# mhauskn/dqn-hfo

Measured on AMD Instinct MI355X. Metric: DQN updates/sec, 1v0 HFO, 4x1024 MLP, minibatch 256, higher is better.
Workload: dtype f32; 1 GPU; BASELINE configs[1]: 1v0 HFO, 1 MI355X, 4x1024 actor-critic, minibatch 256, 1M-transition device replay; replay_transitions=1000000, state_size=58, minibatch=256, minibatch_per_gpu=256, global_minibatch=256, parallelism=single, hip_graph=True, prewarm_updates=992, tuning_flags=0, sampling=on-device Philox, uniform with replacement

## Files before the change

__graft_entry__.py:

```python
import importlib.util
import os
import sys

ROOT = os.path.dirname(os.path.abspath(__file__))


def load_package():
    if "dqn_hfo_amd" in sys.modules:
        return sys.modules["dqn_hfo_amd"]
    pkg_dir = os.path.join(ROOT, "dqn-hfo_amd")
    spec = importlib.util.spec_from_file_location(
        "dqn_hfo_amd", os.path.join(pkg_dir, "__init__.py"), submodule_search_locations=[pkg_dir])
    mod = importlib.util.module_from_spec(spec)
    sys.modules["dqn_hfo_amd"] = mod
    spec.loader.exec_module(mod)
    return mod


def build():
    pkg = load_package()
    lib = pkg.build(verbose=False)
    assert os.path.exists(lib), lib
    if ROOT not in sys.path:
        sys.path.insert(0, ROOT)
    from oracle import c_oracle
    c_oracle.build()
    pkg.capi.load()
    sys.path.insert(0, os.path.join(ROOT, "tests"))
    import testlib
    testlib.load_test()
    from oracle import dropin_build
    if dropin_build.reference_present():
        dropin_build.build(lib)
    return lib


def smoke():
    import numpy as np
    pkg = load_package()
    if ROOT not in sys.path:
        sys.path.insert(0, ROOT)
    sys.path.insert(0, os.path.join(ROOT, "tests"))
    from oracle import c_oracle, torch_ref
    from synth import synth_replay
    rng = np.random.default_rng(7)
    B, S, hid = 32, 59, (128, 64, 64, 64)
    dqn = pkg.DQN(S, minibatch=B, hidden=hid, memory=4096, seed=3)
    orc = c_oracle.Oracle(B=B, S=S, hidden=hid, capacity=4096)
    for net, actor in ((0, True), (1, False)):
        w = torch_ref.init_params_np(rng, S, hid, actor) * 10
        dqn.set_params(net, w); dqn.CloneNet(net)
        orc.set_params(net, w); orc.clone_to_target(net)
    s, a, r, mc, nx, term = synth_replay(rng, 1024, S, mean_len=10)
    dqn.add_transitions_arrays(s, a, r, mc, nx, term)
    orc.add_transitions(s, a, r, mc, nx, term)
    for it in range(3):
        idx = rng.integers(0, 1024, size=B)
        l1, q1 = dqn.UpdateActorCritic(idx)
        l2, q2 = orc.update(idx)
        assert abs(l1 - l2) <= 1e-4 * max(1.0, abs(l2)), (l1, l2)
        assert abs(q1 - q2) <= 1e-4, (q1, q2)
    for net in range(4):
        d = np.abs(dqn.get_params(net) - orc.get_params(net)).max()
# ... 15 lines not shown
```

benchlib/flops.py:

```python


HBM_PEAK_GBS = 8000.0


MFMA_F32_PEAK_TF = 157.3


def tower_weights(in_dim, hidden):
    dims = (in_dim,) + tuple(hidden)
    return [dims[i] * dims[i + 1] for i in range(len(hidden))]


def family_flops(B, S, hidden, shifted=True):
    wa = tower_weights(S, hidden)
    wc = tower_weights(S + 10, hidden)
    h1 = hidden[0]
    L = len(hidden)
    if shifted and L >= 2:
        pair = lambda w: sum(w[j + 1] + w[j] for j in range(1, L - 1))
        return {
            "gemm_fwd_lds_4x2": 2 * B * (2 * sum(wa[1:]) + 2 * sum(wc[1:])),
            "gemm_fwd_lds_2x2": 2 * B * sum(wc[1:]),
            "gemm_fwd_direct": 2 * B * (2 * wa[0] + 3 * wc[0]),
            "gemm_bwd_pair": 2 * B * (pair(wc) + pair(wa)),
            "gemm_dgrad": 2 * B * (sum(wc[1:]) + 10 * h1 + wc[L - 1] + wa[L - 1]),
            "gemm_wgrad": 2 * B * (wc[1] + wc[0] + wa[1] + wa[0]),
        }
    return {
        "gemm_fwd_lds_4x2": 2 * B * (2 * sum(wa[1:]) + 2 * sum(wc[1:])),
        "gemm_fwd_lds_2x2": 2 * B * sum(wc[1:]),
        "gemm_fwd_direct": 2 * B * (2 * wa[0] + 3 * wc[0]),
        "gemm_bwd_pair": 2 * B * (2 * sum(wc[1:]) + 2 * sum(wa[1:])),
        "gemm_dgrad": 2 * B * (sum(wc[1:]) + 10 * h1),
        "gemm_wgrad": 2 * B * (wc[0] + wa[0]),
    }


def family_flops16(B, S, hidden):
    wa = tower_weights(S, hidden)
    wc = tower_weights(S + 10, hidden)
    h1 = hidden[0]
    return {
        "hgemm_fwd": 2 * B * (2 * sum(wa) + 3 * sum(wc)),
        "hgemm_dgrad": 2 * B * (sum(wc[1:]) + sum(wa[1:]) + sum(wc[1:]) + 10 * h1),
        "hgemm_wgrad": 2 * B * (sum(wc) + sum(wa)),
    }


MFMA_F16_PEAK_TF = 2500.0


KERNEL_NAMES = {"hgemm_fwd": "hgemm_nt<2,2>/<1,1> (forward epilogue)", "hgemm_dgrad": "hgemm_nt (dgrad epilogue)",
                "hgemm_wgrad": "hgemm_nt (wgrad epilogue)","gemm_fwd_lds_4x2": "gemm_fwd_lds<4,2,true,1>", "gemm_fwd_lds_2x2": "gemm_fwd_lds<2,2,true,2>",
                "gemm_fwd_direct": "gemm_fwd_direct<4,2>", "gemm_bwd_pair": "gemm_bwd_seq<true>",
                "gemm_dgrad": "gemm_dgrad_lds<1,1>", "gemm_wgrad": "gemm_wgrad_tail<1>"}


TRACE_FAMILY = (("gemm_fwd_lds<4,2,true,1>", "gemm_fwd_lds_4x2"), ("gemm_fwd_lds<4,2,true>", "gemm_fwd_lds_4x2"), ("gemm_fwd_lds<2,2,true", "gemm_fwd_lds_2x2"),
                ("gemm_fwd_lds<1,1,true", "gemm_fwd_lds_2x2"), ("gemm_fwd_direct", "gemm_fwd_direct"), ("gemm_bwd_seq", "gemm_bwd_pair"),
                ("gemm_bwd_pair_direct", "gemm_bwd_pair"), ("gemm_dgrad_lds", "gemm_dgrad"), ("gemm_dgrad_direct", "gemm_dgrad"), ("gemm_dgrad_narrow", "gemm_dgrad"), ("k_dqda_head_bwd", "gemm_dgrad"), ("k_dgrad_qtrain", "gemm_dgrad"),
                ("gemm_wgrad_tail", "gemm_wgrad"), ("gemm_wgrad_narrow", "gemm_wgrad"), ("k_adam_soft", "adam"))
```

dqn-hfo_amd/capi.py:

```python
import ctypes as C
import os

from ._build import LIB, build

MAX_HIDDEN = 8
DP_ID_BYTES = 128
DP_PER_LAYER, DP_HALF_GRADS, DP_SHARD_OPT = 1, 2, 4
DP_UNVERIFIED_OK = 256
TUNE_FP16_WGRAD_PER_LAYER = 1
TUNE_SEPARATE_HEAD_SEED = 2
TUNE_BWD_UNSHIFTED = 4
TUNE_SEPARATE_ACTOR_HEAD_BWD = 8
TUNE_SEPARATE_Q_TRAIN = 16
TUNE_SEPARATE_FIRST_LAYER = 32
TUNE_SEPARATE_CRITIC_FIRST_LAYERS = 64
TUNE_LATE_GATHER = 128
PLAN_FORMS = ("fp16", "data_parallel", "bwd_shifted_critic", "bwd_shifted_actor", "head_wgrad_rides_critic", "head_wgrad_rides_actor",
              "q_train_in_dgrad", "head_seed_fused", "dqda_head_bwd", "critic_l0_rides", "first_layers_merged", "early_gather_l0", "dp_tails_ride", "prioritized")
LOSS_SCALE_STATIC, LOSS_SCALE_DYNAMIC = 0, 1
FP32, FP16 = 0, 1
ACTOR, CRITIC, ACTOR_TARGET, CRITIC_TARGET = 0, 1, 2, 3
KIND_W, KIND_M, KIND_V, KIND_G = 0, 1, 2, 3


class Config(C.Structure):
    _fields_ = [
        ("struct_size", C.c_int32), ("minibatch", C.c_int32), ("state_size", C.c_int32),
        ("num_hidden", C.c_int32), ("hidden", C.c_int32 * MAX_HIDDEN),
        ("replay_capacity", C.c_int32), ("soft_update_freq", C.c_int32),
        ("gamma", C.c_double), ("beta", C.c_double), ("tau", C.c_double),
        ("actor_lr", C.c_float), ("critic_lr", C.c_float), ("momentum", C.c_float),
        ("momentum2", C.c_float), ("delta", C.c_float), ("clip_gradients", C.c_float),
        ("device", C.c_int32), ("dp_world", C.c_int32), ("dp_rank", C.c_int32), ("use_graph", C.c_int32),
        ("seed", C.c_uint64), ("stream", C.c_void_p), ("grad_arena", C.c_void_p),
        ("grad_arena_bytes", C.c_size_t), ("precision", C.c_int32), ("loss_scale", C.c_float),
        ("tuning_flags", C.c_int32),
        ("loss_scale_mode", C.c_int32), ("loss_scale_growth_interval", C.c_int32),
        ("loss_scale_min_mult", C.c_float), ("loss_scale_max_mult", C.c_float),
    ]


class LossScaleState(C.Structure):
    _fields_ = [("struct_size", C.c_int32), ("mode", C.c_int32), ("mult_critic", C.c_float), ("mult_actor", C.c_float),
                ("good_critic", C.c_int32), ("good_actor", C.c_int32), ("backoffs_critic", C.c_int32), ("backoffs_actor", C.c_int32),
                ("growths_critic", C.c_int32), ("growths_actor", C.c_int32), ("skipped_steps", C.c_int32), ("reserved", C.c_int32)]


class UpdatePlan(C.Structure):
    _fields_ = [("struct_size", C.c_int32), ("forms", C.c_int32), ("launches_single", C.c_int32), ("launches_graph_first", C.c_int32),
# ... 169 lines not shown
```

dqn-hfo_amd/csrc/gemm_bodies.hip.h:

```cpp
#pragma once
#include <hip/hip_runtime.h>

#include <cstdint>

#include "learner_args.hip.h"

namespace dqnhip {


__host__ __device__ __forceinline__ void tile_of_counts(int tiles_p, int tiles_q, int b, int& tile_p, int& tile_q) {
  const bool xmap = (tiles_p & 7) == 0;
  const int j = xmap ? b >> 3 : b;
  const int d = j / tiles_q;
  tile_q = j - d * tiles_q;
  tile_p = xmap ? d * 8 + (b & 7) : d;
}
__device__ __forceinline__ void tile_of_problem(const GemmProblem& pr, int b, int& tile_p, int& tile_q) {
  tile_of_counts(pr.tiles_p, pr.tiles_q, b, tile_p, tile_q);
}
__device__ __forceinline__ void tile_of_block(const GemmBatch& batch, int& pi, int& tile_p, int& tile_q) {
  int b = blockIdx.x;
  pi = 0;
#pragma unroll
  for (int i = 1; i < kMaxGroup; ++i)
// ... 370 lines not shown
#define DN_COMPUTE(slot)                                                                \
  { _Pragma("unroll") for (int s = 0; s < 4; ++s) acc[0] = DQN_MFMA((float)rp[slot][s], (float)rq[slot][s], acc[0]); }
  const int nkbN = nkb - nkb % NS;
  if (nkbN > 0) {
#pragma unroll
    for (int i = 0; i < NS; ++i) { DN_LOAD(i, i) DQN_PIN(); }
    int kb = 0;
    for (; kb + NS < nkbN; kb += NS) {
#pragma unroll
      for (int i = 0; i < NS; ++i) { DN_COMPUTE(i) DQN_PIN(); DN_LOAD(i, kb + NS + i) DQN_PIN(); }
    }
#pragma unroll
    for (int i = 0; i < NS; ++i) { DN_COMPUTE(i) }
  }
  for (int kb = nkbN; kb < nkb; ++kb) { DN_LOAD(0, kb) DN_COMPUTE(0) }
#undef DN_LOAD
#undef DN_COMPUTE
  park_accumulators<1>(smem, acc, wave, lane);
  __syncthreads();
  f32x4 v = f32x4{0.f, 0.f, 0.f, 0.f};
  if (wave == 0) v = reduce_accumulator<1>(smem, 0, lane);
  return v;
}
__device__ __forceinline__ void dgrad_narrow_body(const GemmProblem& pr, int tile_p, int tile_q, float* smem) {
  const f32x4 v = dgrad_narrow_tile<4>(pr, tile_p, tile_q, smem);
  if ((threadIdx.x >> 6) == 0) {
    const int lane = threadIdx.x & 63, li = lane & 15, lg = lane >> 4;
    const int q = tile_q * 16 + li, p = tile_p * 16 + (lg << 2);
    *reinterpret_cast<f32x4*>(pr.C + (size_t)q * pr.ldc + p) = v;
  }
}

constexpr int kWgradRing = 4;
template <int TPB, int TQB>
__device__ __forceinline__ void wgrad_direct_body(const GemmProblem& pr, int tile_p, int tile_q, float* smem) {
  constexpr int NACC = TPB * 4 * TQB * 4;
  const int lane = threadIdx.x & 63, wave = threadIdx.x >> 6;
  const int li = lane & 15, lg = lane >> 4;
  const int p0 = tile_p * 64 * TPB, q0 = tile_q * 64 * TQB;
  const int Kw = pr.Kred >> 2;
  const int nst = Kw >> 2;
  const float* pp = pr.P + (size_t)(wave * Kw + lg) * pr.ldp + p0 + li * 4;
  const float* qp = pr.Q + (size_t)(wave * Kw + lg) * pr.ldq + q0 + li * 4;
  const size_t ldp = pr.ldp, ldq = pr.ldq;
  const bool want_db = (pr.db != nullptr) && (tile_p == 0);

  f32x4 acc[NACC];
#pragma unroll
  for (int e = 0; e < NACC; ++e) acc[e] = f32x4{0.f, 0.f, 0.f, 0.f};
  f32x4 dbacc[TQB];
#pragma unroll
  for (int d = 0; d < TQB; ++d) dbacc[d] = f32x4{0.f, 0.f, 0.f, 0.f};
  constexpr int NS = kWgradRing;
  f32x4 rp[NS][TPB], rq[NS][TQB];

#define WG_LOAD(slot, st)                                                               \
  {                                                                                     \
    _Pragma("unroll") for (int b = 0; b < TPB; ++b)                                     \
        rp[slot][b] = *reinterpret_cast<const f32x4*>(pp + (size_t)((st) << 2) * ldp + b * 64); \
    _Pragma("unroll") for (int d = 0; d < TQB; ++d)                                     \
        rq[slot][d] = *reinterpret_cast<const f32x4*>(qp + (size_t)((st) << 2) * ldq + d * 64); \
  }
#define WG_COMPUTE(slot)                                                                \
  {                                                                                     \
    _Pragma("unroll") for (int d = 0; d < TQB; ++d) {                                   \
      dbacc[d].x += rq[slot][d].x; dbacc[d].y += rq[slot][d].y;                         \
      dbacc[d].z += rq[slot][d].z; dbacc[d].w += rq[slot][d].w;                         \
      _Pragma("unroll") for (int qc = 0; qc < 4; ++qc)                                  \
// ... 10 lines not shown
    for (int i = 0; i < NS; ++i) { WG_LOAD(i, i) DQN_PIN(); }
    int st = 0;
    for (; st + NS < nstN; st += NS) {
#pragma unroll
      for (int i = 0; i < NS; ++i) { WG_COMPUTE(i) DQN_PIN(); WG_LOAD(i, st + NS + i) DQN_PIN(); }
    }
#pragma unroll
    for (int i = 0; i < NS; ++i) { WG_COMPUTE(i) }
  }
  {
    const int rem = nst - nstN;
    if (rem > 0) WG_LOAD(0, nstN)
    if (rem > 1) WG_LOAD(1, nstN + 1)
    if (rem > 2) WG_LOAD(2, nstN + 2)
    if (rem > 0) WG_COMPUTE(0)
    if (rem > 1) WG_COMPUTE(1)
    if (rem > 2) WG_COMPUTE(2)
  }
#undef WG_LOAD
#undef WG_COMPUTE

  park_accumulators<NACC>(smem, acc, wave, lane);
  float* sdb = smem + 4 * NACC * 64 * 4;
  if (want_db) {
#pragma unroll
    for (int d = 0; d < TQB; ++d) {
      f32x4 v = dbacc[d];
      v.x += __shfl_xor(v.x, 16, 64); v.y += __shfl_xor(v.y, 16, 64); v.z += __shfl_xor(v.z, 16, 64); v.w += __shfl_xor(v.w, 16, 64);
      v.x += __shfl_xor(v.x, 32, 64); v.y += __shfl_xor(v.y, 32, 64); v.z += __shfl_xor(v.z, 32, 64); v.w += __shfl_xor(v.w, 32, 64);
      if (lg == 0) reinterpret_cast<f32x4*>(sdb)[(wave * TQB + d) * 16 + li] = v;
    }
  }
  __syncthreads();
  float ssq = 0.0f;
#pragma unroll
  for (int g4 = 0; g4 < TQB * 4 * TPB; ++g4) {
    if ((g4 & 3) == wave) {
      const int b = g4 % TPB, dq = g4 / TPB, qc = dq & 3, d = dq >> 2;
      f32x4 r0 = reduce_accumulator<NACC>(smem, g4 * 4 + 0, lane);
      f32x4 r1 = reduce_accumulator<NACC>(smem, g4 * 4 + 1, lane);
      f32x4 r2 = reduce_accumulator<NACC>(smem, g4 * 4 + 2, lane);
      f32x4 r3 = reduce_accumulator<NACC>(smem, g4 * 4 + 3, lane);
      const int n = q0 + d * 64 + (li << 2) + qc;
#pragma unroll
      for (int r = 0; r < 4; ++r) {
        const int p = p0 + b * 64 + (lg << 4) + (r << 2);
        const f32x4 v = f32x4{r0[r], r1[r], r2[r], r3[r]};
        ssq = fmaf(v.x, v.x, ssq); ssq = fmaf(v.y, v.y, ssq); ssq = fmaf(v.z, v.z, ssq); ssq = fmaf(v.w, v.w, ssq);
        *reinterpret_cast<f32x4*>(pr.C + (size_t)n * pr.ldc + p) = v;
      }
    }
  }
  if (want_db && wave == 0 && lane < 16 * TQB) {
    const int d = lane >> 4, l16 = lane & 15;
    const f32x4* s4 = reinterpret_cast<const f32x4*>(sdb);
    const f32x4 a0 = s4[(0 * TQB + d) * 16 + l16], a1 = s4[(1 * TQB + d) * 16 + l16];
    const f32x4 a2 = s4[(2 * TQB + d) * 16 + l16], a3 = s4[(3 * TQB + d) * 16 + l16];
    f32x4 v;
    v.x = (a0.x + a1.x) + (a2.x + a3.x); v.y = (a0.y + a1.y) + (a2.y + a3.y);
    v.z = (a0.z + a1.z) + (a2.z + a3.z); v.w = (a0.w + a1.w) + (a2.w + a3.w);
    *reinterpret_cast<f32x4*>(pr.db + q0 + d * 64 + (l16 << 2)) = v;
    ssq = fmaf(v.x, v.x, ssq); ssq = fmaf(v.y, v.y, ssq); ssq = fmaf(v.z, v.z, ssq); ssq = fmaf(v.w, v.w, ssq);
  }
  if (pr.partial != nullptr) {
    ssq = wave_sum64(ssq);
    __syncthreads();
// ... 461 lines not shown
```

dqn-hfo_amd/csrc/gemm_direct.hip.h:

```cpp
#pragma once
#include <hip/hip_runtime.h>

#include <algorithm>
#include <cstdint>
#include <cstdlib>

#include "gemm_bodies.hip.h"
#include "gemm_plan.hip.h"

namespace dqnhip {

template <int TP, int TQ>
__global__ __launch_bounds__(256) void gemm_fwd_direct(const GemmArgs<kMaxGroup> args) {
  extern __shared__ __attribute__((aligned(16))) float smem[];
  int tile_p, tile_q;
  const GemmProblem pr = problem_of_block(args, tile_p, tile_q);
  fwd_direct_body<TP, TQ>(pr, tile_p, tile_q, smem);
}
template <int TP, int TQ, bool PIN, int NSLOT = 2>
__global__ __launch_bounds__(256) void gemm_fwd_lds(const GemmArgs<kMaxGroup> args) {
  extern __shared__ __attribute__((aligned(16))) float smem[];
  int tile_p, tile_q;
  const GemmProblem pr = problem_of_block(args, tile_p, tile_q);
  fwd_lds_body<TP, TQ, PIN, NSLOT>(pr, tile_p, tile_q, smem);
// ... 50 lines not shown
}
template <int TQD = 1, bool DLDS = false>
__global__ __launch_bounds__(256) void gemm_bwd_pair_direct(const GemmArgs<kMaxGroup> args) {
  extern __shared__ __attribute__((aligned(16))) float smem[];
  int tile_p, tile_q;
  const GemmProblem pr = problem_of_block(args, tile_p, tile_q);
  if (pr.mode == GEMM_WGRAD) wgrad_direct_body<1, 1>(pr, tile_p, tile_q, smem);
  else if constexpr (DLDS) dgrad_lds_body<1, TQD, false>(pr, tile_p, tile_q, smem);
  else dgrad_direct_body<1, TQD>(pr, tile_p, tile_q, smem);
}

template <bool DLDS>
__device__ __forceinline__ void bwd_seq_block(const GemmArgs<2>& args, const int block, float* smem) {
  int tile_p, tile_q;
  HotArgs<2> r;
  const int b = request_args(args, r, block);
  const GemmProblem pw = problem_at<1>(args, r);
  if (b < pw.tiles_p * pw.tiles_q) {
    tile_of_problem(pw, b, tile_p, tile_q);
    wgrad_direct_body<1, 1>(pw, tile_p, tile_q, smem);
  }
  __syncthreads();
  const GemmProblem pd = problem_at<0>(args, r);
  if (b < pd.tiles_p * pd.tiles_q) {
    tile_of_problem(pd, b, tile_p, tile_q);
    if constexpr (DLDS) dgrad_lds_body<1, 1, true>(pd, tile_p, tile_q, smem);
    else dgrad_direct_body<1, 1>(pd, tile_p, tile_q, smem);
  }
}
template <bool DLDS>
__global__ __launch_bounds__(256) void gemm_bwd_seq(const GemmArgs<2> args) {
  extern __shared__ __attribute__((aligned(16))) float smem[];
  bwd_seq_block<DLDS>(args, (int)blockIdx.x, smem);
}

template <int NH>
__global__ __launch_bounds__(256) void gemm_wgrad_narrow_rider(const GemmArgs<kMaxGroup> args, const HeadWgradRider rider) {
  extern __shared__ __attribute__((aligned(16))) float smem[];
  HotArgs<kMaxGroup> r;
  const int b = request_args(args, r, (int)blockIdx.x, rider.blocks);
  if (b < rider.blocks) { head_wgrad_rider<NH>(rider, b, smem); return; }
  int tile_p, tile_q;
  const GemmProblem pr = problem_of_tile(args, r, b - rider.blocks, tile_p, tile_q);
  wgrad_narrow_body<1>(pr, tile_p, tile_q, smem);
}

template <int NH>
__global__ __launch_bounds__(256) void gemm_wgrad_tail(const GemmArgs<2> args, const HeadWgradRider rider, const TailsArgs tails) {
  extern __shared__ __attribute__((aligned(16))) float smem[];
  HotArgs<2> r;
  int blk = request_args(args, r, (int)blockIdx.x, tails.on, rider.blocks);
  int tile_p, tile_q;
  if (tails.on && blk == tails.on - 1) { tails_block(tails, smem, reinterpret_cast<double*>(smem + 8)); return; }
  if (blk < rider.blocks) { head_wgrad_rider<NH>(rider, blk, smem); return; }
  blk -= rider.blocks;
  const int n0 = r.hd.tiles_p[1] * r.hd.tiles_q[1];
  if (blk < n0) { const GemmProblem p0 = problem_at<1>(args, r); tile_of_problem(p0, blk, tile_p, tile_q); wgrad_narrow_body<1>(p0, tile_p, tile_q, smem); return; }
  blk -= n0;
  const GemmProblem p1 = problem_at<0>(args, r);
  tile_of_problem(p1, blk, tile_p, tile_q); wgrad_direct_body<1, 1>(p1, tile_p, tile_q, smem);
}


constexpr int kBwdTileLds = 4 * 16 * 64 * 16 + 4 * 16 * 16;
constexpr int kWgradTailLdsMax = 80 * 1024;

// ... 109 lines not shown
template <int NH>
inline hipError_t wgrad_narrow_rider_launch(GemmBatch& batch, const HeadWgradRider& rider, const LaunchOn& on) {
  const size_t lds = std::max(head_rider_lds_bytes<NH>(rider), (size_t)wgrad_narrow_lds_bytes<1>());
  if (lds > 64 * 1024) return hipErrorInvalidValue;
  tile_batch(batch, 64, 16);
  return packed_launch(gemm_wgrad_narrow_rider<NH>, batch, rider.blocks, (int)lds, on, rider);
}
template <int NH>
inline hipError_t wgrad_tail_launch(GemmBatch& batch, const HeadWgradRider& rider, const LaunchOn& on, const TailsArgs* tails_in = nullptr) {
  TailsArgs tails{}; if (tails_in != nullptr) { tails = *tails_in; tails.on = 1; }
  GemmProblem& w1 = batch.prob[0]; GemmProblem& w0 = batch.prob[1];
  w1.tiles_p = w1.Pdim / 64; w1.tiles_q = w1.Qdim / 64; w1.tile_base = 0;
  w0.tiles_p = w0.Pdim / 64; w0.tiles_q = w0.Qdim / 16; w0.tile_base = w1.tiles_p * w1.tiles_q;
  const int grid = w0.tile_base + w0.tiles_p * w0.tiles_q + rider.blocks + (tails.on ? 1 : 0);
  batch.total_tiles = grid;
  if (tails.on) tails.on = grid;
  const size_t lds = std::max(rider.blocks ? head_rider_lds_bytes<NH>(rider) : (size_t)0, (size_t)kBwdTileLds);
  if (lds > (size_t)kWgradTailLdsMax) return hipErrorInvalidValue;
  GemmArgs<2> args;
  if (batch.n != 2 || !pack_args(batch, args)) return hipErrorInvalidValue;
  return launch(on, gemm_wgrad_tail<NH>, dim3(grid), dim3(256), lds, args, rider, tails);
}
template <bool DLDS>
inline hipError_t bwd_seq_launch(GemmBatch& batch, const LaunchOn& on) {
  GemmProblem& d = batch.prob[0]; GemmProblem& w = batch.prob[1];
  d.tiles_p = d.Pdim / 64; d.tiles_q = d.Qdim / 16; d.tile_base = 0;
  w.tiles_p = w.Pdim / 64; w.tiles_q = w.Qdim / 64; w.tile_base = 0;
  const int nd = d.tiles_p * d.tiles_q, nw = w.tiles_p * w.tiles_q;
  const int grid = nd > nw ? nd : nw;
  batch.total_tiles = grid;
  GemmArgs<2> args;
  if (batch.n != 2 || !pack_args(batch, args, false)) return hipErrorInvalidValue;
  return launch(on, gemm_bwd_seq<DLDS>, dim3(grid), dim3(256), kBwdTileLds, args);
}
template <int UNUSED = 0>
inline hipError_t gemm_form_launch(int form, GemmBatch& b, const LaunchOn& on, const HeadWgradRider* rider = nullptr, const TailsArgs* tails = nullptr) {
  if (!gemm_form_accepts(form, b)) return hipErrorInvalidValue;
  const bool tail = form == GEMM_FORM_WGRAD_TAIL_1 || form == GEMM_FORM_WGRAD_TAIL_NO;
  if (!tail && (rider != nullptr || tails != nullptr)) return hipErrorInvalidValue;
  const HeadWgradRider no_rider{};
  switch (form) {
    case GEMM_FORM_FWD_DIRECT_2x2: return fwd_direct_launch<2, 2>(b, on);
    case GEMM_FORM_FWD_DIRECT_4x2: return fwd_direct_launch<4, 2>(b, on);
    case GEMM_FORM_FWD_LDS_1x1: return fwd_lds_launch<1, 1, true>(b, on);
    case GEMM_FORM_FWD_LDS_2x2: return fwd_lds_launch<2, 2, true>(b, on);
    case GEMM_FORM_FWD_LDS_4x2: return fwd_lds_launch<4, 2, true>(b, on);
    case GEMM_FORM_FWD_LDS_4x2_ONE_IMAGE: return fwd_lds_launch<4, 2, true, 1>(b, on);
    case GEMM_FORM_DGRAD_DIRECT: return dgrad_direct_launch<1, 1>(b, on);
    case GEMM_FORM_DGRAD_LDS: return dgrad_lds_launch<1, 1>(b, on);
    case GEMM_FORM_DGRAD_NARROW: return dgrad_narrow_launch(b, on);
    case GEMM_FORM_WGRAD_NARROW: return wgrad_narrow_launch<1>(b, on);
    case GEMM_FORM_BWD_SEQ: return bwd_seq_launch<false>(b, on);
    case GEMM_FORM_BWD_SEQ_LDS: return bwd_seq_launch<true>(b, on);
    case GEMM_FORM_BWD_PAIR: return bwd_pair_direct_launch<1, false>(b, on);
    case GEMM_FORM_BWD_PAIR_LDS: return bwd_pair_direct_launch<1, true>(b, on);
    case GEMM_FORM_WGRAD_TAIL_1: return wgrad_tail_launch<1>(b, rider ? *rider : no_rider, on, tails);
    case GEMM_FORM_WGRAD_TAIL_NO: return wgrad_tail_launch<kNO>(b, rider ? *rider : no_rider, on, tails);
  }
  return hipErrorInvalidValue;
}
template <typename K>
inline hipError_t direct_prepare(K kernel, int lds_bytes) {
  return hipFuncSetAttribute(reinterpret_cast<const void*>(kernel), hipFuncAttributeMaxDynamicSharedMemorySize, lds_bytes);
}
template <int UNUSED = 0>
inline hipError_t direct_prepare_all() {
  hipError_t e = direct_prepare(gemm_bwd_seq<true>, kBwdTileLds);
  if (e == hipSuccess) e = direct_prepare(gemm_bwd_seq<false>, kBwdTileLds);
  if (e == hipSuccess) e = direct_prepare(gemm_wgrad_tail<1>, kWgradTailLdsMax);
  if (e == hipSuccess) e = direct_prepare(gemm_wgrad_tail<10>, kWgradTailLdsMax);
  if (e == hipSuccess) e = direct_prepare(gemm_bwd_pair_direct<1, true>, kBwdTileLds);
  if (e == hipSuccess) e = direct_prepare(gemm_bwd_pair_direct<1, false>, kBwdTileLds);
  if (e == hipSuccess) e = direct_prepare(gemm_fwd_lds<4, 2, true>, fwd_lds_bytes<4, 2, true>());
  return e;
}

}
```

dqn-hfo_amd/csrc/gemm_plan.hip.h:

```cpp
#pragma once
#include "gemm_common.hip.h"

namespace dqnhip {

enum GemmForm {
  GEMM_FORM_FWD_DIRECT_2x2 = 0, GEMM_FORM_FWD_DIRECT_4x2 = 1,
  GEMM_FORM_FWD_LDS_1x1 = 2, GEMM_FORM_FWD_LDS_2x2 = 3, GEMM_FORM_FWD_LDS_4x2 = 4, GEMM_FORM_FWD_LDS_4x2_ONE_IMAGE = 5,
  GEMM_FORM_DGRAD_DIRECT = 6, GEMM_FORM_DGRAD_LDS = 7, GEMM_FORM_DGRAD_NARROW = 8, GEMM_FORM_WGRAD_NARROW = 9,
  GEMM_FORM_BWD_SEQ = 10, GEMM_FORM_BWD_SEQ_LDS = 11,
  GEMM_FORM_BWD_PAIR = 12, GEMM_FORM_BWD_PAIR_LDS = 13,
  GEMM_FORM_WGRAD_TAIL_1 = 14, GEMM_FORM_WGRAD_TAIL_NO = 15,
  GEMM_FORM_COUNT = 16
};
enum GemmFormKind { GEMM_KIND_FWD_DIRECT, GEMM_KIND_FWD_LDS, GEMM_KIND_DGRAD, GEMM_KIND_DGRAD_NARROW, GEMM_KIND_WGRAD_NARROW,
                    GEMM_KIND_BWD , GEMM_KIND_TAIL };
struct GemmFormSpec { GemmFormKind kind; int bp, bq; bool lds; int n_min, n_max; const char* name; };
inline constexpr GemmFormSpec kGemmForms[GEMM_FORM_COUNT] = {
    {GEMM_KIND_FWD_DIRECT, 32, 32, false, 1, kMaxGroup, "fwd_direct<2,2>"},
    {GEMM_KIND_FWD_DIRECT, 64, 32, false, 1, kMaxGroup, "fwd_direct<4,2>"},
    {GEMM_KIND_FWD_LDS, 16, 16, true, 1, kMaxGroup, "fwd_lds<1,1,true>"},
    {GEMM_KIND_FWD_LDS, 32, 32, true, 1, kMaxGroup, "fwd_lds<2,2,true>"},
    {GEMM_KIND_FWD_LDS, 64, 32, true, 1, kMaxGroup, "fwd_lds<4,2,true>"},
    {GEMM_KIND_FWD_LDS, 64, 32, true, 1, kMaxGroup, "fwd_lds<4,2,true,1>"},
    {GEMM_KIND_DGRAD, 64, 16, false, 1, kMaxGroup, "dgrad_direct<1,1>"},
// ... 19 lines not shown
inline bool gemm_fwd_accepts(const GemmProblem& p, const GemmFormSpec& f) {
  if (p.mode != GEMM_FWD || !gemm_tiles_ok(p, f.bp, f.bq) || !gemm_kred_ok(p.Kred, f.lds)) return false;
  if (p.mask || p.db || p.partial) return false;
  if (p.xcopy_dst && (f.lds || p.xcopy_n <= 0 || p.xcopy_col < 0 || (long)p.xcopy_col + p.xcopy_n > p.ldp)) return false;
  return !p.seed_w == !p.C2 && !p.dot_w == !p.dot_out;
}
inline bool gemm_dgrad_accepts(const GemmProblem& p, bool lds, bool narrow) {
  if (p.mode != GEMM_DGRAD || !gemm_tiles_ok(p, narrow ? 16 : 64, 16) || !gemm_kred_ok(p.Kred, lds)) return false;
  return gemm_fwd_extras_absent(p) && !p.db && !p.partial;
}
inline bool gemm_wgrad_accepts(const GemmProblem& p, bool narrow) {
  if (p.mode != GEMM_WGRAD || !gemm_tiles_ok(p, 64, narrow ? 16 : 64) || p.Kred < 16 || p.Kred % 16) return false;
  return gemm_fwd_extras_absent(p) && !p.mask;
}
inline bool gemm_form_accepts(int form, const GemmBatch& b) {
  if (form < 0 || form >= GEMM_FORM_COUNT) return false;
  const GemmFormSpec& f = kGemmForms[form];
  if (b.n < f.n_min || b.n > f.n_max) return false;
  switch (f.kind) {
    case GEMM_KIND_FWD_DIRECT: case GEMM_KIND_FWD_LDS:
      for (int i = 0; i < b.n; ++i) if (!gemm_fwd_accepts(b.prob[i], f)) return false;
      return true;
    case GEMM_KIND_DGRAD: case GEMM_KIND_DGRAD_NARROW:
      for (int i = 0; i < b.n; ++i) if (!gemm_dgrad_accepts(b.prob[i], f.lds, f.kind == GEMM_KIND_DGRAD_NARROW)) return false;
      return true;
    case GEMM_KIND_WGRAD_NARROW:
      for (int i = 0; i < b.n; ++i) if (!gemm_wgrad_accepts(b.prob[i], true)) return false;
      return true;
    case GEMM_KIND_BWD: return gemm_dgrad_accepts(b.prob[0], f.lds, false) && gemm_wgrad_accepts(b.prob[1], false);
    case GEMM_KIND_TAIL: return gemm_wgrad_accepts(b.prob[0], false) && gemm_wgrad_accepts(b.prob[1], true);
  }
  return false;
}

inline GemmForm fwd_form(int kred, int pdim, int rows, int n) {
  const bool lds = gemm_lds_ok(kred);
  if (n == 1) {
    if (lds && rows <= 128) return GEMM_FORM_FWD_LDS_1x1;
    if (lds && rows >= 512 && pdim % 64 == 0) return GEMM_FORM_FWD_LDS_4x2;
    return lds ? GEMM_FORM_FWD_LDS_2x2 : GEMM_FORM_FWD_DIRECT_2x2;
  }
  const long t42 = (long)n * (pdim / 64) * (rows / 32), t22 = (long)n * (pdim / 32) * (rows / 32);
  if (lds) {
    if (t42 >= 192) return GEMM_FORM_FWD_LDS_4x2_ONE_IMAGE;
    if (t22 >= 128 || rows > 128 || rows % 16) return GEMM_FORM_FWD_LDS_2x2;
    return GEMM_FORM_FWD_LDS_1x1;
  }
  return t42 >= 64 ? GEMM_FORM_FWD_DIRECT_4x2 : GEMM_FORM_FWD_DIRECT_2x2;
}
inline GemmForm first_layers_form() { return GEMM_FORM_FWD_DIRECT_4x2; }

inline bool bwd_layer_is_pair(int kp_in, int out, int rows) {
  const long tiles = (long)(kp_in / 64) * (rows / 16) + (long)(kp_in / 64) * (out / 64);
  return tiles <= 256 && rows % 16 == 0 && kp_in % 64 == 0 && out % 64 == 0;
}
inline GemmForm dgrad_form(int out, bool narrow = false) {
  return narrow ? GEMM_FORM_DGRAD_NARROW : (gemm_lds_ok(out) ? GEMM_FORM_DGRAD_LDS : GEMM_FORM_DGRAD_DIRECT);
}
inline GemmForm wgrad_form() { return GEMM_FORM_WGRAD_NARROW; }
inline GemmForm bwd_form(int kp_in, int out, int rows) {
  if (bwd_layer_is_pair(kp_in, out, rows)) return gemm_lds_ok(out) ? GEMM_FORM_BWD_PAIR_LDS : GEMM_FORM_BWD_PAIR;
  return gemm_lds_ok(out) ? GEMM_FORM_BWD_SEQ_LDS : GEMM_FORM_BWD_SEQ;
}
inline GemmForm bwd_shifted_mid_form(int out) { return gemm_lds_ok(out) ? GEMM_FORM_BWD_SEQ_LDS : GEMM_FORM_BWD_SEQ; }
inline GemmForm bwd_shifted_tail_form(int nh) { return nh == 1 ? GEMM_FORM_WGRAD_TAIL_1 : GEMM_FORM_WGRAD_TAIL_NO; }

}
```

dqn-hfo_amd/csrc/learner.hip:

```cpp
#include "learner_internal.hip.h"
#include "gemm_direct.hip.h"
#include "hgemm.hip.h"
#include "head_fwd_kernels.hip.h"
#include "head_kernels.hip.h"
#include "small_kernels.hip.h"

using namespace dqnhip;
using namespace dqnhip_host;

namespace dqnhip_host {

const char* const kFamily[kNumFamily] = {"gemm_fwd_lds_4x2", "gemm_dgrad", "gemm_wgrad", "adam", "gemm_bwd_pair", "gemm_fwd_lds_2x2", "gemm_fwd_direct",
                                         "hgemm_fwd", "hgemm_dgrad", "hgemm_wgrad",
                                         "per_sync", "per_sample", "per_update"};
static Family family_of(GemmForm f, int n) {
  switch (kGemmForms[f].kind) {
    case GEMM_KIND_FWD_DIRECT: return kFamFwdDirect;
    case GEMM_KIND_FWD_LDS: return n == 1 ? kFamFwdLds2x2 : kFamFwdLds4x2;
    case GEMM_KIND_DGRAD: case GEMM_KIND_DGRAD_NARROW: return kFamDgrad;
    case GEMM_KIND_BWD: return kFamBwdPair;
    case GEMM_KIND_WGRAD_NARROW: case GEMM_KIND_TAIL: break;
  }
  return kFamWgrad;
}
// ... 43 lines not shown
    p.P = wat(h, net, l.w_off[i]); p.ldp = l.kp[i];
    p.Q = dZ[i + 1]; p.ldq = l.kp[i + 1];
    p.C = dZ[i]; p.ldc = l.kp[i];
    p.Pdim = l.kp[i]; p.Qdim = rows; p.Kred = l.dims[i + 1];
    p.mask = i > 0 ? act[i] : nullptr; p.ldm = l.kp[i];
    return p;
  };
  auto wgrad_of = [&](int i) {
    GemmProblem p{};
    p.mode = GEMM_WGRAD;
    p.P = act[i]; p.ldp = l.kp[i];
    p.Q = dZ[i + 1]; p.ldq = l.kp[i + 1];
    p.C = garena + l.w_off[i]; p.ldc = l.kp[i];
    p.Pdim = l.kp[i]; p.Qdim = l.dims[i + 1]; p.Kred = rows;
    p.db = garena + l.b_off[i];
    p.partial = partial ? partial + l.part_off[i] : nullptr;
    return p;
  };
  auto layer_slice = [&](int i) { return (i + 1 < l.L ? l.w_off[i + 1] : l.hw_off) - l.w_off[i]; };
  const bool shifted = want_w && !input_grad && bwd_is_shifted(h, l, rows);
  if (r.qtrain != nullptr && !(shifted && dgrad_form(l.dims[l.L]) == GEMM_FORM_DGRAD_LDS)) return fail("internal: k_dgrad_qtrain needs the shifted schedule and an LDS-staged top layer");
  if (shifted) {
    {
      GemmBatch bd{}; bd.n = 1; bd.prob[0] = dgrad_of(l.L - 1);
      const GemmForm f = dgrad_form(l.dims[l.L]);
      if (r.qtrain != nullptr) {
        bd.prob[0].Q = r.qtrain_seed;
        RC(form_check(f, bd));
        HIPCHK(dgrad_qtrain_launch(bd, *r.qtrain, timed(h, family_of(f, 1), st)));
      } else RC(form_launch(h, st, f, bd));
    }
    for (int i = l.L - 2; i >= 1; --i) {
      GemmBatch b{}; b.n = 2; b.prob[0] = dgrad_of(i); b.prob[1] = wgrad_of(i + 1);
      RC(form_launch(h, st, bwd_shifted_mid_form(l.dims[i + 1]), b));
      if (h->comm && h->dp_per_layer) RC(dp_reduce_slice(h, st, net, l.w_off[i + 1], layer_slice(i + 1)));
    }
    {
      GemmBatch b{}; b.n = 2; b.prob[0] = wgrad_of(1); b.prob[1] = wgrad_of(0);
      RC(form_launch(h, st, bwd_shifted_tail_form(l.NH), b, r.rider, r.tails));
      if (h->comm && h->dp_per_layer) RC(dp_reduce_slice(h, st, net, l.w_off[0], layer_slice(0) + layer_slice(1)));
    }
    if (qrider) return fail("internal: the q-head rider found no carrier launch");
    return 0;
  }
  if (r.tails != nullptr) return fail("internal: the tails block rides in the shifted schedule's last launch only");
  for (int i = l.L - 1; i >= 0; --i) {
    GemmBatch bd{}, bw{};
    const bool need_dx = (i > 0 || input_grad);
    if (need_dx) bd.prob[bd.n++] = dgrad_of(i);
    if (want_w) bw.prob[bw.n++] = wgrad_of(i);
    if (need_dx && want_w) {
      GemmBatch b{}; b.n = 2; b.prob[0] = bd.prob[0]; b.prob[1] = bw.prob[0];
      RC(form_launch(h, st, bwd_form(l.kp[i], l.dims[i + 1], rows), b));
    } else if (need_dx && i == 0 && r.fuse != nullptr) {
      GemmProblem p = bd.prob[0];
      p.P += r.in_lo; p.C = nullptr; p.Pdim = 16; p.mask = nullptr;
      r.fuse->pr = p;
      const QHeadRider none{};
      HIPCHK(dqda_head_bwd_launch(*r.fuse, qrider ? *qrider : none, timed(h, kFamDgrad, st)));
      qrider = nullptr;
    } else if (need_dx && i == 0 && r.in_hi > r.in_lo && rows % 16 == 0) {
      GemmProblem& p = bd.prob[0];
      const int c0 = (r.in_lo / 16) * 16, c1 = std::min(l.kp[0], (r.in_hi + 15) / 16 * 16);
      p.P += c0; p.C += c0; p.Pdim = c1 - c0;
      if (p.mask) p.mask += c0;
      const GemmForm f = dgrad_form(l.dims[1], true);
      if (qrider) {
// ... 636 lines not shown
```

include/dqnhip.h:

```cpp
#ifndef DQNHIP_H_
#define DQNHIP_H_

#include <stddef.h>
#include <stdint.h>

#ifdef __cplusplus
extern "C" {
#endif

#define DQNHIP_ACTION_SIZE 4
#define DQNHIP_ACTION_PARAM_SIZE 6
#define DQNHIP_ACTOR_OUT 10
#define DQNHIP_MAX_HIDDEN 8

enum dqnhip_net {
  DQNHIP_ACTOR = 0,
  DQNHIP_CRITIC = 1,
  DQNHIP_ACTOR_TARGET = 2,
  DQNHIP_CRITIC_TARGET = 3
};

enum dqnhip_param_kind {
  DQNHIP_KIND_W = 0,
  DQNHIP_KIND_M = 1,
// ... 18 lines not shown
  double beta;
  double tau;
  float actor_lr;
  float critic_lr;
  float momentum;
  float momentum2;
  float delta;
  float clip_gradients;
  int32_t device;
  int32_t dp_world;
  int32_t dp_rank;
  int32_t use_graph;
  uint64_t seed;
  void* stream;
  void* grad_arena;
  size_t grad_arena_bytes;
  int32_t precision;
  float loss_scale;
  int32_t tuning_flags;
  int32_t loss_scale_mode;
  int32_t loss_scale_growth_interval;
  float loss_scale_min_mult;
  float loss_scale_max_mult;
} dqnhip_config;

#define DQNHIP_TUNE_FP16_WGRAD_PER_LAYER 1
#define DQNHIP_TUNE_SEPARATE_HEAD_SEED 2
#define DQNHIP_TUNE_BWD_UNSHIFTED 4
#define DQNHIP_TUNE_SEPARATE_ACTOR_HEAD_BWD 8
#define DQNHIP_TUNE_SEPARATE_Q_TRAIN 16
#define DQNHIP_TUNE_SEPARATE_FIRST_LAYER 32
#define DQNHIP_TUNE_SEPARATE_CRITIC_FIRST_LAYERS 64
#define DQNHIP_TUNE_LATE_GATHER 128

typedef struct dqnhip_learner* dqnhip_handle;

void dqnhip_default_config(dqnhip_config* cfg, int32_t state_size);

size_t dqnhip_grad_arena_bytes(const dqnhip_config* cfg);

const char* dqnhip_last_error(void);

int dqnhip_create(const dqnhip_config* cfg, dqnhip_handle* out);
int dqnhip_destroy(dqnhip_handle h);


int dqnhip_update(dqnhip_handle h, const int32_t* idx_host,
                  float* critic_loss, float* avg_q);

int dqnhip_update_pipelined(dqnhip_handle h, const int32_t* idx_host,
                            float* critic_loss, float* avg_q);

int dqnhip_update_chained(dqnhip_handle h, const int32_t* idx_host, const int32_t* idx_next,
                          float* critic_loss, float* avg_q);

int dqnhip_update_async(dqnhip_handle h, const int32_t* idx_host);

int dqnhip_update_async_n(dqnhip_handle h, int32_t n);

int dqnhip_update_indexed_n(dqnhip_handle h, const int32_t* idx_host , int32_t n);

int dqnhip_collect_stats(dqnhip_handle h, float* critic_loss , float* avg_q ,
                         int32_t cap, int32_t* n_out);

int dqnhip_update_phase(dqnhip_handle h, int32_t phase, const int32_t* idx_host);
int dqnhip_update_abort(dqnhip_handle h);
// ... 199 lines not shown
```

Before: 3614 updates/s.

## Add wide-tile fused dgrad/wgrad kernel for shifted backward middle layers

Adds a new kernel for the middle layers of the shifted backward schedule. Each launch runs a dgrad on 64x32 tiles and a wgrad on 128x64 tiles, with dgrad and wgrad blocks interleaved in groups of eight. This replaces the gemm_bwd_seq form whenever the tile count stays at or below 256, which is meant to fill the GPU better for 1024-wide layers. The wgrad epilogue gets a per-half sum-of-squares variant that writes more gradient-norm partials per tile, and a tuning flag restores the old sequential form.

After: 3648 updates/s, median of 6. About the same (+0.9%).

```diff
diff --git a/__graft_entry__.py b/__graft_entry__.py
--- a/__graft_entry__.py
+++ b/__graft_entry__.py
@@ -29,6 +29,8 @@
     sys.path.insert(0, os.path.join(ROOT, "tests"))
     import testlib
     testlib.load_test()
+    import bwd_wide_lib
+    bwd_wide_lib.load()
     from oracle import dropin_build
     if dropin_build.reference_present():
         dropin_build.build(lib)
diff --git a/benchlib/flops.py b/benchlib/flops.py
--- a/benchlib/flops.py
+++ b/benchlib/flops.py
@@ -52,7 +52,7 @@
 
 KERNEL_NAMES = {"hgemm_fwd": "hgemm_nt<2,2>/<1,1> (forward epilogue)", "hgemm_dgrad": "hgemm_nt (dgrad epilogue)",
                 "hgemm_wgrad": "hgemm_nt (wgrad epilogue)","gemm_fwd_lds_4x2": "gemm_fwd_lds<4,2,true,1>", "gemm_fwd_lds_2x2": "gemm_fwd_lds<2,2,true,2>",
-                "gemm_fwd_direct": "gemm_fwd_direct<4,2>", "gemm_bwd_pair": "gemm_bwd_seq<true>",
+                "gemm_fwd_direct": "gemm_fwd_direct<4,2>", "gemm_bwd_pair": "gemm_bwd_pair_direct_wide<0>",
                 "gemm_dgrad": "gemm_dgrad_lds<1,1>", "gemm_wgrad": "gemm_wgrad_tail<1>"}
 
 
diff --git a/dqn-hfo_amd/capi.py b/dqn-hfo_amd/capi.py
--- a/dqn-hfo_amd/capi.py
+++ b/dqn-hfo_amd/capi.py
@@ -15,6 +15,7 @@
 TUNE_SEPARATE_FIRST_LAYER = 32
 TUNE_SEPARATE_CRITIC_FIRST_LAYERS = 64
 TUNE_LATE_GATHER = 128
+TUNE_BWD_MID_SEQ = 256
 PLAN_FORMS = ("fp16", "data_parallel", "bwd_shifted_critic", "bwd_shifted_actor", "head_wgrad_rides_critic", "head_wgrad_rides_actor",
               "q_train_in_dgrad", "head_seed_fused", "dqda_head_bwd", "critic_l0_rides", "first_layers_merged", "early_gather_l0", "dp_tails_ride", "prioritized")
 LOSS_SCALE_STATIC, LOSS_SCALE_DYNAMIC = 0, 1
diff --git a/dqn-hfo_amd/csrc/gemm_bodies.hip.h b/dqn-hfo_amd/csrc/gemm_bodies.hip.h
--- a/dqn-hfo_amd/csrc/gemm_bodies.hip.h
+++ b/dqn-hfo_amd/csrc/gemm_bodies.hip.h
@@ -426,8 +426,9 @@
 }
 
 constexpr int kWgradRing = 4;
-template <int TPB, int TQB>
+template <int TPB, int TQB, bool HALVES = false>
 __device__ __forceinline__ void wgrad_direct_body(const GemmProblem& pr, int tile_p, int tile_q, float* smem) {
+  static_assert(!HALVES || (TPB == 2 && TQB == 1), "the per-half epilogue is the 128 x 64 tile's");
   constexpr int NACC = TPB * 4 * TQB * 4;
   const int lane = threadIdx.x & 63, wave = threadIdx.x >> 6;
   const int li = lane & 15, lg = lane >> 4;
@@ -504,6 +505,50 @@
     }
   }
   __syncthreads();
+  if constexpr (HALVES) {
+    float ssq2[TPB];
+#pragma unroll
+    for (int b = 0; b < TPB; ++b) {
+      ssq2[b] = 0.0f;
+      const int g4 = wave * TPB + b;
+      f32x4 r0 = reduce_accumulator<NACC>(smem, g4 * 4 + 0, lane);
+      f32x4 r1 = reduce_accumulator<NACC>(smem, g4 * 4 + 1, lane);
+      f32x4 r2 = reduce_accumulator<NACC>(smem, g4 * 4 + 2, lane);
+      f32x4 r3 = reduce_accumulator<NACC>(smem, g4 * 4 + 3, lane);
+      const int n = q0 + (li << 2) + wave;
+#pragma unroll
+      for (int r = 0; r < 4; ++r) {
+        const int p = p0 + b * 64 + (lg << 4) + (r << 2);
+        const f32x4 v = f32x4{r0[r], r1[r], r2[r], r3[r]};
+        ssq2[b] = fmaf(v.x, v.x, ssq2[b]); ssq2[b] = fmaf(v.y, v.y, ssq2[b]); ssq2[b] = fmaf(v.z, v.z, ssq2[b]); ssq2[b] = fmaf(v.w, v.w, ssq2[b]);
+        *reinterpret_cast<f32x4*>(pr.C + (size_t)n * pr.ldc + p) = v;
+      }
+    }
+    if (want_db && wave == 0 && lane < 16) {
+      const f32x4* s4 = reinterpret_cast<const f32x4*>(sdb);
+      const f32x4 a0 = s4[0 * 16 + lane], a1 = s4[1 * 16 + lane], a2 = s4[2 * 16 + lane], a3 = s4[3 * 16 + lane];
+      f32x4 v;
+      v.x = (a0.x + a1.x) + (a2.x + a3.x); v.y = (a0.y + a1.y) + (a2.y + a3.y);
+      v.z = (a0.z + a1.z) + (a2.z + a3.z); v.w = (a0.w + a1.w) + (a2.w + a3.w);
+      *reinterpret_cast<f32x4*>(pr.db + q0 + (lane << 2)) = v;
+      ssq2[0] = fmaf(v.x, v.x, ssq2[0]); ssq2[0] = fmaf(v.y, v.y, ssq2[0]); ssq2[0] = fmaf(v.z, v.z, ssq2[0]); ssq2[0] = fmaf(v.w, v.w, ssq2[0]);
+    }
+    if (pr.partial != nullptr) {
+#pragma unroll
+      for (int b = 0; b < TPB; ++b) ssq2[b] = wave_sum64(ssq2[b]);
+      __syncthreads();
+      if (lane == 0) {
+#pragma unroll
+        for (int b = 0; b < TPB; ++b) smem[b * 4 + wave] = ssq2[b];
+      }
+      __syncthreads();
+      if ((int)threadIdx.x < TPB) {
+        const int b = threadIdx.x;
+        pr.partial[tile_q * (pr.tiles_p * TPB) + tile_p * TPB + b] = (smem[b * 4 + 0] + smem[b * 4 + 1]) + (smem[b * 4 + 2] + smem[b * 4 + 3]);
+      }
+    }
+    return;
+  }
   float ssq = 0.0f;
 #pragma unroll
   for (int g4 = 0; g4 < TQB * 4 * TPB; ++g4) {
diff --git a/dqn-hfo_amd/csrc/gemm_direct.hip.h b/dqn-hfo_amd/csrc/gemm_direct.hip.h
--- a/dqn-hfo_amd/csrc/gemm_direct.hip.h
+++ b/dqn-hfo_amd/csrc/gemm_direct.hip.h
@@ -106,6 +106,28 @@
 __global__ __launch_bounds__(256) void gemm_bwd_seq(const GemmArgs<2> args) {
   extern __shared__ __attribute__((aligned(16))) float smem[];
   bwd_seq_block<DLDS>(args, (int)blockIdx.x, smem);
+}
+
+template <int UNUSED = 0>
+__global__ __launch_bounds__(256) void gemm_bwd_pair_direct_wide(const GemmArgs<2> args) {
+  extern __shared__ __attribute__((aligned(16))) float smem[];
+  int tile_p, tile_q;
+  HotArgs<2> r;
+  const int b = request_args(args, r, (int)blockIdx.x);
+  const int nd = r.hd.tiles_p[0] * r.hd.tiles_q[0], nw = r.hd.tiles_p[1] * r.hd.tiles_q[1];
+  const int m8 = (nd < nw ? nd : nw) & ~7;
+  bool is_w; int k;
+  if (b < 2 * m8) { const int j = b >> 3; is_w = (j & 1) == 0; k = ((j >> 1) << 3) + (b & 7); }
+  else { const int t = b - 2 * m8; is_w = t < nw - m8; k = m8 + (is_w ? t : t - (nw - m8)); }
+  if (is_w) {
+    const GemmProblem pw = problem_at<1>(args, r);
+    tile_of_problem(pw, k, tile_p, tile_q);
+    wgrad_direct_body<2, 1, true>(pw, tile_p, tile_q, smem);
+  } else {
+    const GemmProblem pd = problem_at<0>(args, r);
+    tile_of_problem(pd, k, tile_p, tile_q);
+    dgrad_lds_body<1, 2, true>(pd, tile_p, tile_q, smem);
+  }
 }
 
 template <int NH>
@@ -281,6 +303,19 @@
   GemmArgs<2> args;
   if (batch.n != 2 || !pack_args(batch, args, false)) return hipErrorInvalidValue;
   return launch(on, gemm_bwd_seq<DLDS>, dim3(grid), dim3(256), kBwdTileLds, args);
+}
+constexpr int kBwdWideLds = 4 * 32 * 64 * 16 + 4 * 16 * 16;
+template <int UNUSED = 0>
+inline hipError_t bwd_wide_pair_launch(GemmBatch& batch, const LaunchOn& on) {
+  if (!gemm_bwd_wide_accepts(batch)) return hipErrorInvalidValue;
+  GemmProblem& d = batch.prob[0]; GemmProblem& w = batch.prob[1];
+  d.tiles_p = d.Pdim / 64; d.tiles_q = d.Qdim / 32; d.tile_base = 0;
+  w.tiles_p = w.Pdim / 128; w.tiles_q = w.Qdim / 64; w.tile_base = 0;
+  const int grid = d.tiles_p * d.tiles_q + w.tiles_p * w.tiles_q;
+  batch.total_tiles = grid;
+  GemmArgs<2> args;
+  if (!pack_args(batch, args, false)) return hipErrorInvalidValue;
+  return launch(on, gemm_bwd_pair_direct_wide<0>, dim3(grid), dim3(256), kBwdWideLds, args);
 }
 template <int UNUSED = 0>
 inline hipError_t gemm_form_launch(int form, GemmBatch& b, const LaunchOn& on, const HeadWgradRider* rider = nullptr, const TailsArgs* tails = nullptr) {
@@ -321,6 +356,7 @@
   if (e == hipSuccess) e = direct_prepare(gemm_bwd_pair_direct<1, true>, kBwdTileLds);
   if (e == hipSuccess) e = direct_prepare(gemm_bwd_pair_direct<1, false>, kBwdTileLds);
   if (e == hipSuccess) e = direct_prepare(gemm_fwd_lds<4, 2, true>, fwd_lds_bytes<4, 2, true>());
+  if (e == hipSuccess) e = direct_prepare(gemm_bwd_pair_direct_wide<0>, kBwdWideLds);
   return e;
 }
 
diff --git a/dqn-hfo_amd/csrc/gemm_plan.hip.h b/dqn-hfo_amd/csrc/gemm_plan.hip.h
--- a/dqn-hfo_amd/csrc/gemm_plan.hip.h
+++ b/dqn-hfo_amd/csrc/gemm_plan.hip.h
@@ -75,6 +75,13 @@
   }
   return false;
 }
+inline bool gemm_bwd_wide_accepts(const GemmBatch& b) {
+  if (b.n != 2 || !gemm_dgrad_accepts(b.prob[0], true, false) || !gemm_wgrad_accepts(b.prob[1], false)) return false;
+  return b.prob[0].Qdim % 32 == 0 && b.prob[1].Pdim % 128 == 0;
+}
+inline long bwd_wide_tiles(int d_pdim, int d_rows, int w_pdim, int w_qdim) {
+  return (long)(w_pdim / 128) * (w_qdim / 64) + (long)(d_pdim / 64) * (d_rows / 32);
+}
 
 inline GemmForm fwd_form(int kred, int pdim, int rows, int n) {
   const bool lds = gemm_lds_ok(kred);
@@ -106,6 +113,14 @@
   return gemm_lds_ok(out) ? GEMM_FORM_BWD_SEQ_LDS : GEMM_FORM_BWD_SEQ;
 }
 inline GemmForm bwd_shifted_mid_form(int out) { return gemm_lds_ok(out) ? GEMM_FORM_BWD_SEQ_LDS : GEMM_FORM_BWD_SEQ; }
+inline bool bwd_shifted_mid_is_wide(int kp_in, int out, int rows, int kp_above, int out_above) {
+  if (kp_in <= 0 || out <= 0 || rows <= 0 || kp_above <= 0 || out_above <= 0) return false;
+  if (kp_in % 64 || !gemm_lds_ok(out) || rows % 32 || kp_above % 128 || out_above % 64) return false;
+  return bwd_wide_tiles(kp_in, rows, kp_above, out_above) <= 256;
+}
+inline bool bwd_shifted_mid_is_wide(int kp_in, int out, int rows) {
+  return kp_in % 128 == 0 && !bwd_layer_is_pair(kp_in, out, rows) && bwd_shifted_mid_is_wide(kp_in, out, rows, kp_in, out);
+}
 inline GemmForm bwd_shifted_tail_form(int nh) { return nh == 1 ? GEMM_FORM_WGRAD_TAIL_1 : GEMM_FORM_WGRAD_TAIL_NO; }
 
 }
diff --git a/dqn-hfo_amd/csrc/learner.hip b/dqn-hfo_amd/csrc/learner.hip
--- a/dqn-hfo_amd/csrc/learner.hip
+++ b/dqn-hfo_amd/csrc/learner.hip
@@ -99,7 +99,9 @@
     }
     for (int i = l.L - 2; i >= 1; --i) {
       GemmBatch b{}; b.n = 2; b.prob[0] = dgrad_of(i); b.prob[1] = wgrad_of(i + 1);
-      RC(form_launch(h, st, bwd_shifted_mid_form(l.dims[i + 1]), b));
+      if (!(h->cfg.tuning_flags & DQNHIP_TUNE_BWD_MID_SEQ) && bwd_shifted_mid_is_wide(l.kp[i], l.dims[i + 1], rows, l.kp[i + 1], l.dims[i + 2]))
+        HIPCHK(bwd_wide_pair_launch(b, timed(h, kFamBwdPair, st)));
+      else RC(form_launch(h, st, bwd_shifted_mid_form(l.dims[i + 1]), b));
       if (h->comm && h->dp_per_layer) RC(dp_reduce_slice(h, st, net, l.w_off[i + 1], layer_slice(i + 1)));
     }
     {
diff --git a/include/dqnhip.h b/include/dqnhip.h
--- a/include/dqnhip.h
+++ b/include/dqnhip.h
@@ -74,6 +74,7 @@
 #define DQNHIP_TUNE_SEPARATE_FIRST_LAYER 32
 #define DQNHIP_TUNE_SEPARATE_CRITIC_FIRST_LAYERS 64
 #define DQNHIP_TUNE_LATE_GATHER 128
+#define DQNHIP_TUNE_BWD_MID_SEQ 256
 
 typedef struct dqnhip_learner* dqnhip_handle;
 
```
